# DerrickWang005/CRIS.pytorch

Hardware: AMD Instinct MI355X
Metric: train-step samples/sec, CRIS-R50 416x416 bs=64; loss parity vs ref (higher is better)
Workload: dtype bf16; 1 GPU; CRIS-R50 bf16 training step (fwd+BCE+bwd+Adam), 416x416, per-GPU bs=8, 17-token text, synthetic RefCOCO-shape batch resident in HBM (BASELINE.json configs[1]); global_batch=8, parallelism=dp1, launch=graph, graph_captured=True, syncbn_exchange=none, grad_exchange=none

## Files before the change

### cris/pytorch_amd/csrc/api.hip

```cpp
#include "common.h"
#include "../../../include/cris_hip.h"
#include <stdarg.h>
#include <string.h>

static thread_local char g_err[512] = {0};

void cris_set_error(const char* fmt, ...) {
    va_list ap;
    va_start(ap, fmt);
    vsnprintf(g_err, sizeof(g_err), fmt, ap);
    va_end(ap);
}

extern "C" const char* cris_last_error(void) { return g_err; }
extern "C" int cris_abi_version(void) { return CRIS_ABI_VERSION; }

extern "C" int cris_sizeof(const char* name) {
#define S(n) if (!strcmp(name, #n)) return (int)sizeof(n)
    S(cris_conv_gemm_params);
    S(cris_wgrad_params);
    S(cris_conv_gemm_group);
    S(cris_wgrad_group);
    S(cris_pack_desc);
    S(cris_conv_gemm_fp8_params);
    S(cris_pack_fp8_desc);
    S(cris_bn_apply_params);
    S(cris_bn_bwd_params);
    S(cris_ln_fwd_params);
    S(cris_ln_bwd_params);
    S(cris_sum_entry);
    S(cris_sum_group);
    S(cris_attn_params);
    S(cris_adam_desc);
    S(cris_ema_desc);
    S(cris_p2p_params);
    S(cris_p2p_link);
    S(cris_p2p_arena_params);
    S(cris_zero_ranges);
    S(cris_sample_desc);
    S(cris_eval_desc);
    S(cris_jpeg_info);
    S(cris_jpeg_image);
#undef S
    return -1;
// ... 51 lines not shown
```

### cris/pytorch_amd/csrc/norm.hip

```cpp
#include "common.h"
#include "../../../include/cris_hip.h"
#include "p2p_ll.h"
#include <string.h>

#define BN_WIDE_MIN 128
#define BN_MERGE_MIN 512
#define BN_MERGE_SLICES 64

template <int PL>
__device__ __forceinline__ float bn_lane_sum(float (*sh)[17], float v, int pl, int cl) {
    __syncthreads();
    sh[pl][cl] = v;
    __syncthreads();
    if (PL == 64) {
        float g = 0.f;
        if (pl < 8) {
#pragma unroll
            for (int j = 0; j < 8; ++j) g += sh[pl * 8 + j][cl];
        }
        __syncthreads();
        if (pl < 8) sh[pl][cl] = g;
        __syncthreads();
    }
    float t = sh[0][cl];
// ... 1000 lines not shown
                if (in_relu && !(v[i][j] > 0.f)) m = 0.f;
                if (in_thresh) m = cris_keep(in_key, row * (uint32_t)C + (uint32_t)(c0 + j), in_thresh) ? m * in_scale : 0.f;
                v[i][j] *= m;
                if (WANT_MASK) mask_out[i][j] = m;
            }
        } else {
#pragma unroll
            for (int j = 0; j < 8; ++j) {
                v[i][j] = 0.f;
                if (WANT_MASK) mask_out[i][j] = 0.f;
            }
        }
    }
}

__global__ __launch_bounds__(256) void ln_fwd_kernel(const cris_ln_fwd_params p) {
    const int lane = threadIdx.x & 63;
    const int wave_g = blockIdx.x * 4 + (threadIdx.x >> 6);
    const int nwaves = gridDim.x * 4;
    const uint32_t sdev = p.seed_dev ? p.seed_dev[0] : 0u;
    const uint32_t in_key = cris_drop_key(p.in_seed + sdev, p.in_stream);
    const uint32_t out_key = cris_drop_key(p.out_seed + sdev, p.out_stream);
    const float in_scale = p.in_thresh ? 1.f / (1.f - p.in_drop_p) : 1.f;
    const float out_scale = p.out_thresh ? 1.f / (1.f - p.out_drop_p) : 1.f;
    const float invC = 1.f / (float)p.C;
    for (int row = wave_g; row < p.rows; row += nwaves) {
        float v[LN_MAXV][8];
        ln_load_row<false>(p.x, p.x_f32, (size_t)row * p.ldx, p.C, lane, p.in_relu, p.in_thresh, in_scale, in_key, (uint32_t)row,
                           v, v);
        float s = 0.f;
#pragma unroll
        for (int i = 0; i < LN_MAXV; ++i)
#pragma unroll
            for (int j = 0; j < 8; ++j) s += v[i][j];
        const float mean = wave_sum(s) * invC;
        float q = 0.f;
#pragma unroll
        for (int i = 0; i < LN_MAXV; ++i) {
            const int c0 = (lane + 64 * i) * 8;
            if (c0 < p.C) {
#pragma unroll
                for (int j = 0; j < 8; ++j) {
                    const float d = v[i][j] - mean;
                    q += d * d;
                }
            }
        }
        const float rstd = rsqrtf(wave_sum(q) * invC + p.eps);
        if (lane == 0) {
            p.mean[row] = mean;
            p.rstd[row] = rstd;
        }
#pragma unroll
        for (int i = 0; i < LN_MAXV; ++i) {
            const int c0 = (lane + 64 * i) * 8;
            if (c0 >= p.C) continue;
            float ga[8], be[8], o[8];
            load8f(p.gamma + c0, ga);
            load8f(p.beta + c0, be);
#pragma unroll
            for (int j = 0; j < 8; ++j) o[j] = (v[i][j] - mean) * rstd * ga[j] + be[j];
            const size_t oo = (size_t)row * p.C + c0;
            if (p.y) cris_st16(p.y + oo, pack8(o));
            if (p.ypos) {
                float pe[8], t[8];
                load8f(p.pos + (size_t)(row % p.pos_rows) * p.C + c0, pe);
#pragma unroll
                for (int j = 0; j < 8; ++j) t[j] = o[j] + pe[j];
                cris_st16(p.ypos + oo, pack8(t));
            }
            if (p.out_f32) {
                float r[8];
                if (p.resid) load8f(p.resid + oo, r);
                else {
#pragma unroll
                    for (int j = 0; j < 8; ++j) r[j] = 0.f;
                }
#pragma unroll
                for (int j = 0; j < 8; ++j) {
                    float t = o[j];
                    if (p.out_thresh) t = cris_keep(out_key, (uint32_t)row * (uint32_t)p.C + (uint32_t)(c0 + j), p.out_thresh) ? t * out_scale : 0.f;
                    r[j] += t;
                }
                *reinterpret_cast<float4*>(p.out_f32 + oo) = make_float4(r[0], r[1], r[2], r[3]);
                *reinterpret_cast<float4*>(p.out_f32 + oo + 4) = make_float4(r[4], r[5], r[6], r[7]);
            }
        }
    }
}

extern "C" int cris_ln_fwd(const cris_ln_fwd_params* pp, void* stream) {
    const cris_ln_fwd_params& p = *pp;
    CRIS_CHECK_ARG(p.x && p.gamma && p.beta && p.mean && p.rstd && p.rows > 0, "null operand");
    CRIS_CHECK_ARG((p.C & 7) == 0 && p.C <= 64 * 8 * LN_MAXV && (p.ldx & 7) == 0, "C must be a multiple of 8, <= 2048");
    CRIS_CHECK_ARG(!p.ypos || (p.pos && p.pos_rows > 0), "ypos needs pos");
    CRIS_CHECK_ARG((long)p.rows * p.C < (1L << 32), "dropout index overflow");
    const int grid = cris_grid_1d(p.rows, 4, 2048);
    hipLaunchKernelGGL(ln_fwd_kernel, dim3(grid), dim3(256), 0, (hipStream_t)stream, p);
    CRIS_LAUNCH_CHECK();
    return 0;
}

template <int V>
__global__ __launch_bounds__(256) void ln_bwd_kernel(const cris_ln_bwd_params p) {
    __shared__ float sg[2][64 * 8 * V];
    const int lane = threadIdx.x & 63;
    const int wave_g = blockIdx.x * 4 + (threadIdx.x >> 6);
    const int nwaves = gridDim.x * 4;
    for (int i = threadIdx.x; i < 2 * 64 * 8 * V; i += 256) (&sg[0][0])[i] = 0.f;
    __syncthreads();
    const uint32_t sdev = p.seed_dev ? p.seed_dev[0] : 0u;
    const uint32_t in_key = cris_drop_key(p.in_seed + sdev, p.in_stream);
    const uint32_t out_key = cris_drop_key(p.out_seed + sdev, p.out_stream);
    const float in_scale = p.in_thresh ? 1.f / (1.f - p.in_drop_p) : 1.f;
    const float out_scale = p.out_thresh ? 1.f / (1.f - p.out_drop_p) : 1.f;
// ... 27 lines not shown
                if (p.dypos) {
                    load8bf(p.dypos + oo, t);
#pragma unroll
                    for (int j = 0; j < 8; ++j) g[j] += t[j];
                }
                if (p.dout_f32) {
                    load8f(p.dout_f32 + oo, t);
#pragma unroll
                    for (int j = 0; j < 8; ++j) {
                        float d = t[j];
                        if (p.out_thresh) d = cris_keep(out_key, (uint32_t)row * (uint32_t)p.C + (uint32_t)(c0 + j), p.out_thresh) ? d * out_scale : 0.f;
                        g[j] += d;
                    }
                }
                load8f(p.gamma + c0, ga);
#pragma unroll
                for (int j = 0; j < 8; ++j) {
                    const float xh = (v[i][j] - mean) * rstd;
                    v[i][j] = xh;
                    dga[i][j] += g[j] * xh;
                    dbe[i][j] += g[j];
                    a[i][j] = g[j] * ga[j];
                    s1 += a[i][j];
                    s2 += a[i][j] * xh;
                }
            } else {
#pragma unroll
                for (int j = 0; j < 8; ++j) a[i][j] = 0.f;
            }
        }
        const float m1 = wave_sum(s1) * invC, m2 = wave_sum(s2) * invC;
#pragma unroll
        for (int i = 0; i < V; ++i) {
            const int c0 = (lane + 64 * i) * 8;
            if (c0 >= p.C) continue;
            float o[8];
#pragma unroll
            for (int j = 0; j < 8; ++j) o[j] = rstd * (a[i][j] - m1 - v[i][j] * m2) * msk[i][j];
            const size_t xo = (size_t)row * p.ldx + c0;
            if (p.dx_f32) {
                float* d = reinterpret_cast<float*>(p.dx) + xo;
                if (p.dx_accum) {
                    float old[8];
                    load8f(d, old);
#pragma unroll
                    for (int j = 0; j < 8; ++j) o[j] += old[j];
                }
                *reinterpret_cast<float4*>(d) = make_float4(o[0], o[1], o[2], o[3]);
                *reinterpret_cast<float4*>(d + 4) = make_float4(o[4], o[5], o[6], o[7]);
            } else {
                cris_st16(reinterpret_cast<bf16_t*>(p.dx) + xo, pack8(o));
            }
        }
    }
    for (int w = 0; w < 4; ++w) {
        if ((int)(threadIdx.x >> 6) == w) {
#pragma unroll
            for (int i = 0; i < V; ++i) {
                const int c0 = (lane + 64 * i) * 8;
                if (c0 < p.C) {
#pragma unroll
                    for (int j = 0; j < 8; ++j) {
                        sg[0][c0 + j] += dga[i][j];
                        sg[1][c0 + j] += dbe[i][j];
                    }
                }
            }
        }
        __syncthreads();
    }
    float* part = p.part + (size_t)blockIdx.x * 2 * p.C;
    for (int c = threadIdx.x; c < p.C; c += 256) {
        part[c] = sg[0][c];
        part[p.C + c] = sg[1][c];
    }
}

constexpr int LN_BWD_BLOCKS = 512;
static int ln_bwd_grid(int rows) { return cris_grid_1d(rows, 4, LN_BWD_BLOCKS); }
extern "C" int cris_ln_bwd_parts(int rows) { return ln_bwd_grid(rows); }

extern "C" int cris_ln_bwd(const cris_ln_bwd_params* pp, void* stream) {
    const cris_ln_bwd_params& p = *pp;
    CRIS_CHECK_ARG(p.x && p.gamma && p.mean && p.rstd && p.dx && p.part && p.rows > 0, "null operand");
    CRIS_CHECK_ARG(p.dy || p.dypos || p.dout_f32, "no incoming gradient");
    CRIS_CHECK_ARG((p.C & 7) == 0 && p.C <= 64 * 8 * LN_MAXV && (p.ldx & 7) == 0, "C must be a multiple of 8, <= 2048");
    CRIS_CHECK_ARG(!p.dx_accum || p.dx_f32, "accumulate only into fp32");
    static const int narrow = cris_env_int("CRIS_LN_BWD_V", 1);
    const dim3 grid(ln_bwd_grid(p.rows));
    if (narrow && p.C <= 512) hipLaunchKernelGGL(ln_bwd_kernel<1>, grid, dim3(256), 0, (hipStream_t)stream, p);
    else if (narrow && p.C <= 1024) hipLaunchKernelGGL(ln_bwd_kernel<2>, grid, dim3(256), 0, (hipStream_t)stream, p);
    else hipLaunchKernelGGL(ln_bwd_kernel<LN_MAXV>, grid, dim3(256), 0, (hipStream_t)stream, p);
    CRIS_LAUNCH_CHECK();
    return 0;
}

__global__ __launch_bounds__(256) void sum_group_kernel(const cris_sum_group g) {
    __shared__ float sh[4][64];
    int ei = 0;
#pragma unroll
    for (int i = 1; i < CRIS_SUM_GROUP_MAX; ++i) ei += g.block_start[i] <= (int)blockIdx.x ? 1 : 0;
    const cris_sum_entry e = g.e[ei];
    const int cl = threadIdx.x & 63, pl = threadIdx.x >> 6;
    const int c = (blockIdx.x - g.block_start[ei]) * 64 + cl;
    float a = 0.f;
    if (c < e.ncol)
        for (int i = pl; i < e.nparts; i += 4) a += e.part[(size_t)i * e.ld + c];
    sh[pl][cl] = a;
    __syncthreads();
    if (pl == 0 && c < e.ncol) e.out[c] = (sh[0][cl] + sh[1][cl]) + (sh[2][cl] + sh[3][cl]);
}
// ... 16 lines not shown
```

### cris/pytorch_amd/engine.py

```python
from __future__ import annotations

from typing import Callable, Dict, List, Optional

import torch
from torch import nn

from . import debug, ops, tables
from .arch import ClipSpec, HeadSpec, build_param_tree
from .ops import BF16, Drop, Geom, NO_DROP, pad8, pad32

F32 = torch.float32
BN_EPS, BN_MOM, LN_EPS = 1e-5, 0.1, 1e-5


class Act:
    __slots__ = ("t", "Bn", "H", "W", "C", "ld", "coff", "root", "_g", "aux")
    _engine = None

    def __init__(self, t, Bn, H, W, C, ld=None, coff=0, root=None):
        self.t, self.Bn, self.H, self.W, self.C = t, Bn, H, W, C
        self.ld = ld if ld is not None else C
        self.coff = coff
        self.root = root if root is not None else self
        self._g = None
# ... 443 lines not shown
                        ops.axpy_f32(resid.root._g, outs.g, 1.0)
                if dx_stream is not None:
                    dx, accum = dx_stream.grad_target()
                else:
                    dx, acc = x.grad_target()
                    accum = False
                    assert not acc, "bf16 LN input gradient cannot be accumulated"
                ops.ln_bwd(x.t, gamma, mean, rstd, rows, C, dx, ldx=x.ld, dy=None if (y is None or y.g is None) else y.g,
                           dypos=None if (ypos is None or ypos.g is None) else ypos.g,
                           dout_f32=None if outs is None else outs.g, dgamma=self.G[pfx + ".weight"], dbeta=self.G[pfx + ".bias"],
                           dx_accum=accum, in_relu=in_relu, in_drop=in_drop, out_drop=out_drop, queue=self._sq)

            self.tape.append(bwd)
        return y, ypos, outs

    def new_T(self, B, Hn, L, secs=1):
        Lpad = pad32(L)
        buf = self.zeros(secs, B * Hn * 64, Lpad, dtype=BF16)
        return dict(buf=buf, L=L, Lpad=Lpad, E=Hn * 64, sec_stride=B * Hn * 64 * Lpad)

    def attention(self, q: Act, k: Act, v: Act, Qt, Kt, Vt, B, Hn, Lq, Lk, *, causal=False, key_tokens=None, drop: Drop = NO_DROP):
        E = Hn * 64
        o = self.new_act(B, Lq, 1, E)
        lse = self.empty(B * Hn, Lq, dtype=F32)
        Lkp, Lqp = pad32(Lk), pad32(Lq)
        qv, kv, vv = q.t[:, q.coff:], k.t[:, k.coff:], v.t[:, v.coff:]
        prm = ops.attn_params(qv, kv, vv, Vt, B, Hn, Lq, Lk, Lkp, 64 ** -0.5, ldq=q.ld, ldk=k.ld, ldv=v.ld, Kt=Kt, Qt=Qt,
                              Lq_pad=Lqp, key_tokens=key_tokens, causal=causal, drop=drop)
        ops.attn_fwd(prm, o.t, lse, ldo=o.ld)
        if self.training:
# ... 329 lines not shown
                gx, acc = txt.grad_target()
                ops.add_bf16(txtpos.g, gx, txt.M, txt.C, b=gx if acc else None)
            self.tape.append(bwd_txtpos)
        for i in range(hd.num_layers):
            p = "decoder.layers.%d" % i
            v2, qk, _ = self.ln(vis, p + ".norm1", pos=vpos, pos_rows=HW, dx_stream=vis)
            T2, Tv = self.new_T(B, Hn, HW, secs=2), self.new_T(B, Hn, HW)
            G = self.group_begin()
            qkp = self.gemm(qk, p + ".self_attn.in_proj_weight", 2 * C, rows=(0, 2 * C), bias=p + ".self_attn.in_proj_bias", outT=T2, group=G)
            vp = self.gemm(v2, p + ".self_attn.in_proj_weight", C, rows=(2 * C, 3 * C), bias=p + ".self_attn.in_proj_bias", outT=Tv, group=G)
            self.group_end(G)
            o, dOt = self.attention(qkp.slice(0, C), qkp.slice(C, C), vp, T2["buf"][0], T2["buf"][1], Tv["buf"][0], B, Hn, HW, HW,
                                    drop=self.drop(i, 0))
            a = self.gemm(o, p + ".self_attn.out_proj.weight", C, bias=p + ".self_attn.out_proj.bias")
            self._patch_outT_on_dgrad(dOt)
            _, _, vis1 = self.ln(a, p + ".self_attn_norm", want_y=False, resid=vis, out_drop=self.drop(i, 1))
            _, qc, _ = self.ln(vis1, p + ".norm2", want_y=False, pos=vpos, pos_rows=HW, dx_stream=vis1)
            Tq, Tk, Tvv = self.new_T(B, Hn, HW), self.new_T(B, Hn, L), self.new_T(B, Hn, L)
            m = p + ".multihead_attn"
            G = self.group_begin()
            qx = self.gemm(qc, m + ".in_proj_weight", C, rows=(0, C), bias=m + ".in_proj_bias", outT=Tq, group=G)
            kx = self.gemm(txtpos, m + ".in_proj_weight", C, rows=(C, 2 * C), bias=m + ".in_proj_bias", outT=Tk, group=G)
            vx = self.gemm(txt, m + ".in_proj_weight", C, rows=(2 * C, 3 * C), bias=m + ".in_proj_bias", outT=Tvv, group=G)
            self.group_end(G)
            o2, dOt2 = self.attention(qx, kx, vx, Tq["buf"][0], Tk["buf"][0], Tvv["buf"][0], B, Hn, HW, L, key_tokens=word,
                                      drop=self.drop(i, 2))
            a2 = self.gemm(o2, m + ".out_proj.weight", C, bias=m + ".out_proj.bias")
            self._patch_outT_on_dgrad(dOt2)
            _, _, vis2 = self.ln(a2, p + ".cross_attn_norm", want_y=False, resid=vis1, out_drop=self.drop(i, 3))
            h3, _, _ = self.ln(vis2, p + ".norm3", dx_stream=vis2)
            u = self.gemm(h3, p + ".ffn.0.weight", hd.dim_ffn, bias=p + ".ffn.0.bias")
            hn, _, _ = self.ln(u, p + ".ffn.3", in_relu=True, in_drop=self.drop(i, 4))
            vis3 = self.new_act(B, H, W, C, dtype=F32)
            self.gemm(hn, p + ".ffn.4.weight", C, bias=p + ".ffn.4.bias", out=vis3, resid=vis2, drop=self.drop(i, 5), stream_grad=vis3)
            self._link_stream(vis3, vis2)
            vis = vis3
        out, _, _ = self.ln(vis, "decoder.norm", dx_stream=vis)
        if self.training:
            def bwd_in():
                gx, acc = fq.grad_target()
                assert not acc
                ops.cast_f32_bf16(vis0.g, gx)
            self.tape.insert(self._dec_tape_start, bwd_in)
        return out

# ... 187 lines not shown
```

### cris/pytorch_amd/hip.py

```python
import contextlib
import ctypes as C
import os

import torch

_HERE = os.path.dirname(os.path.abspath(__file__))
LIB_PATH = os.path.join(_HERE, "csrc", "libcris_hip.so")
if os.environ.get("CRIS_LIB_VARIANT"):
    LIB_PATH = os.path.join(_HERE, "csrc", "variants", "libcris_hip_%s.so" % os.environ["CRIS_LIB_VARIANT"])

P, I, L, F, U = C.c_void_p, C.c_int, C.c_long, C.c_float, C.c_uint32


class ConvGemmParams(C.Structure):
    _fields_ = [("A", P), ("Wt", P), ("bias", P), ("resid", P), ("out", P), ("outT", P), ("colsum", P), ("colsq", P),
                ("T_sec_stride", L),
                ("lda", I), ("a_coff", I),
                ("Bn", I), ("H", I), ("W", I), ("C", I),
                ("OH", I), ("OW", I), ("KH", I), ("KW", I), ("stride", I), ("pad", I),
                ("ldb", I),
                ("M", I), ("N", I), ("K", I),
                ("act", I),
                ("ldr", I), ("r_coff", I), ("resid_f32", I),
                ("ldc", I), ("c_coff", I), ("out_f32", I),
# ... 99 lines not shown
                ("out_drop_p", F), ("out_thresh", U), ("out_seed", U), ("out_stream", U),
                ("eps", F),
                ("seed_dev", P)]


class LnBwdParams(C.Structure):
    _fields_ = [("x", P), ("x_f32", I), ("ldx", I),
                ("gamma", P),
                ("mean", P), ("rstd", P),
                ("dy", P), ("dypos", P), ("dout_f32", P),
                ("part", P),
                ("dx", P), ("dx_f32", I), ("dx_accum", I),
                ("rows", I), ("C", I),
                ("in_relu", I),
                ("in_drop_p", F), ("in_thresh", U), ("in_seed", U), ("in_stream", U),
                ("out_drop_p", F), ("out_thresh", U), ("out_seed", U), ("out_stream", U),
                ("seed_dev", P)]


class AttnParams(C.Structure):
    _fields_ = [("Q", P), ("ldq", I),
                ("K", P), ("ldk", I),
                ("V", P), ("ldv", I),
                ("Vt", P), ("Kt", P), ("Qt", P), ("Lk_pad", I), ("Lq_pad", I),
                ("key_tokens", P),
                ("O", P), ("ldo", I),
                ("lse", P),
                ("dO", P), ("lddo", I), ("dOt", P),
                ("delta", P),
                ("dQ", P), ("lddq", I),
# ... 77 lines not shown

class P2PLink(C.Structure):
    _fields_ = [("boxes", P), ("err", P), ("gen_dev", P),
                ("gen_host", I), ("rank", I), ("world", I),
                ("slot", I), ("slots", I), ("max_floats", I), ("spin_limit", I)]


class P2PArenaParams(C.Structure):
    _fields_ = [("arenas", P), ("lo", C.c_long), ("n", C.c_long), ("link", P2PLink), ("blocks", I)]


STRUCTS = {
    "cris_conv_gemm_params": ConvGemmParams, "cris_conv_gemm_group": ConvGemmGroup, "cris_wgrad_params": WgradParams, "cris_wgrad_group": WgradGroup, "cris_pack_desc": PackDesc,
    "cris_conv_gemm_fp8_params": ConvGemmFp8Params, "cris_pack_fp8_desc": PackFp8Desc,
    "cris_bn_apply_params": BnApplyParams, "cris_bn_bwd_params": BnBwdParams, "cris_ln_fwd_params": LnFwdParams,
    "cris_ln_bwd_params": LnBwdParams, "cris_sum_entry": SumEntry, "cris_sum_group": SumGroup, "cris_attn_params": AttnParams, "cris_adam_desc": AdamDesc, "cris_ema_desc": EmaDesc, "cris_p2p_params": P2PParams, "cris_p2p_link": P2PLink, "cris_p2p_arena_params": P2PArenaParams, "cris_zero_ranges": ZeroRanges,
    "cris_sample_desc": SampleDesc, "cris_eval_desc": EvalDesc, "cris_jpeg_info": JpegInfo, "cris_jpeg_image": JpegImage,
}

_SIGS = {
    "cris_last_error": (C.c_char_p, []),
    "cris_abi_version": (I, []),
    "cris_sizeof": (I, [C.c_char_p]),
    "cris_echo_conv_gemm": (L, [P]),
    "cris_conv_gemm": (I, [P, P]),
    "cris_conv_wgrad": (I, [P, P]),
    "cris_conv_wgrad_group": (I, [P, P]),
    "cris_conv_wgrad_tile": (I, [P]),
    "cris_wgrad_reduce": (I, [P, P]),
    "cris_wgrad_reduce_group": (I, [P, P]),
    "cris_wgrad_ws_floats": (L, [I, I, I, I]),
# ... 18 lines not shown
    "cris_absmax_ws_floats": (I, []),
    "cris_bn_partials_rows": (I, [I]),
    "cris_bn_finalize": (I, [P, P, I, I, F, F, P, P, P, P, F, F, I, P, P, P, P, P, P, P]),
    "cris_bn_sync_pack": (I, [P, P, P, F, I, P]),
    "cris_bn_sync_unpack": (I, [P, P, F, I, P]),
    "cris_colstats_bf16": (I, [P, I, I, I, I, I, P, P, P]),
    "cris_bn_eval_coeffs": (I, [P, P, P, P, F, I, P, P, P]),
    "cris_bn_apply": (I, [P, P]),
    "cris_bn_bwd_reduce": (I, [P, P]),
    "cris_bn_bwd_apply": (I, [P, P]),
    "cris_bn_bwd_ws_floats": (L, [P]),
    "cris_ln_bwd_parts": (I, [I]),
    "cris_sum_tables": (I, [P, P]),
    "cris_ln_fwd": (I, [P, P]),
    "cris_ln_bwd": (I, [P, P]),
    "cris_attn_fwd": (I, [P, P]),
    "cris_attn_bwd_dq": (I, [P, P]),
    "cris_attn_bwd_dkv": (I, [P, P]),
    "cris_attn_plan": (I, [P, I]),
    "cris_stem_im2col": (I, [P, I, I, I, P, P]),
    "cris_avgpool2_fwd": (I, [P, I, I, I, I, I, I, P, I, I, P]),
    "cris_avgpool2_bwd": (I, [P, I, I, I, I, I, I, P, I, I, I, P]),
    "cris_upsample2_fwd": (I, [P, I, I, I, I, I, I, P, I, I, P]),
    "cris_upsample2_bwd": (I, [P, I, I, I, I, I, I, P, I, I, I, P]),
    "cris_fill_coords": (I, [P, I, I, I, I, I, I, P]),
    "cris_gather_samples_bf16": (I, [P, I, I, P, I, I, I, P, I, I, P]),
    "cris_add_bf16": (I, [P, I, I, P, I, I, P, I, I, I, I, P]),
    "cris_add_rowtable": (I, [P, I, P, I, P, I, I, I, P]),
    "cris_cast_f32_bf16": (I, [P, P, L, P]),
    "cris_cast_bf16_f32": (I, [P, P, L, I, P]),
# ... 181 lines not shown
```

### cris/pytorch_amd/ops.py

```python
from __future__ import annotations

import ctypes as C
import math
import os
from dataclasses import dataclass
from typing import Optional

import torch

from . import hip
from .hip import ptr

BF16 = torch.bfloat16


def _stream():
    return torch.cuda.current_stream().cuda_stream


def pad8(n: int) -> int:
    return (n + 7) // 8 * 8


def pad32(n: int) -> int:
# ... 568 lines not shown
    p.dx, p.dx_f32, p.dx_accum = ptr(dx), int(dx.dtype == torch.float32), int(dx_accum)
    p.rows, p.C, p.in_relu = rows, C_, int(in_relu)
    p.in_drop_p, p.in_thresh, p.in_seed, p.in_stream = in_drop.p, in_drop.thresh, in_drop.seed & 0xFFFFFFFF, in_drop.stream
    p.out_drop_p, p.out_thresh, p.out_seed, p.out_stream = out_drop.p, out_drop.thresh, out_drop.seed & 0xFFFFFFFF, out_drop.stream
    p.seed_dev = ptr(in_drop.dev if in_drop.dev is not None else out_drop.dev)
    hip.call("cris_ln_bwd", C.byref(p), _stream())
    q = queue if queue is not None else SumQueue()
    if dgamma is not None:
        q.add(part, dgamma, nparts, C_, 2 * C_, 0)
    if dbeta is not None:
        q.add(part, dbeta, nparts, C_, 2 * C_, C_)
    if queue is None:
        q.flush()


def attn_params(Q, K, V, Vt, B, Hn, Lq, Lk, Lk_pad, scale, *, ldq=None, ldk=None, ldv=None, Kt=None, Qt=None, Lq_pad=0,
                key_tokens=None, causal=False, drop: Drop = NO_DROP):
    p = hip.AttnParams()
    p.Q, p.ldq = ptr(Q), ldq if ldq is not None else Q.shape[-1]
    p.K, p.ldk = ptr(K), ldk if ldk is not None else K.shape[-1]
    p.V, p.ldv = ptr(V), ldv if ldv is not None else V.shape[-1]
    p.Vt, p.Kt, p.Qt, p.Lk_pad, p.Lq_pad = ptr(Vt), ptr(Kt), ptr(Qt), Lk_pad, Lq_pad
    p.key_tokens = ptr(key_tokens)
    p.B, p.Hn, p.Lq, p.Lk, p.causal, p.scale = B, Hn, Lq, Lk, int(causal), float(scale)
    p.drop_p, p.drop_thresh, p.drop_seed, p.drop_stream = drop.p, drop.thresh, drop.seed & 0xFFFFFFFF, drop.stream
    p.drop_seed_dev = ptr(drop.dev)
    return p


def attn_fwd(p, O, lse, ldo=None):
# ... 666 lines not shown
```

### include/cris_hip.h

```cpp
#ifndef CRIS_HIP_H
#define CRIS_HIP_H
#include <stddef.h>
#include <stdint.h>
#ifdef __cplusplus
extern "C" {
#endif

typedef uint16_t cris_bf16;

const char* cris_last_error(void);
#define CRIS_ABI_VERSION 8
int cris_abi_version(void);
int cris_sizeof(const char* struct_name);
long cris_echo_conv_gemm(const void* conv_gemm_params);

typedef struct {
    const cris_bf16* A;
    const cris_bf16* Wt;
    const float* bias;
    const void* resid;
    void* out;
    cris_bf16* outT;
    float* colsum;
    float* colsq;
// ... 191 lines not shown
    const float* gamma;
    const float* mean; const float* rstd;
    const cris_bf16* dy;
    const cris_bf16* dypos;
    const float* dout_f32;
    float* part;
    void* dx; int dx_f32; int dx_accum;
    int rows, C;
    int in_relu;
    float in_drop_p; uint32_t in_thresh, in_seed, in_stream;
    float out_drop_p; uint32_t out_thresh, out_seed, out_stream;
    const uint32_t* seed_dev;
} cris_ln_bwd_params;
int cris_ln_bwd(const cris_ln_bwd_params* p, void* stream);
int cris_ln_bwd_parts(int rows);

#define CRIS_SUM_GROUP_MAX 64
typedef struct { const float* part; float* out; int nparts, ncol, ld, pad_; } cris_sum_entry;
typedef struct {
    int n;
    int block_start[CRIS_SUM_GROUP_MAX + 1];
    cris_sum_entry e[CRIS_SUM_GROUP_MAX];
} cris_sum_group;
int cris_sum_tables(const cris_sum_group* g, void* stream);

typedef struct {
    const cris_bf16* Q;  int ldq;
    const cris_bf16* K;  int ldk;
    const cris_bf16* V;  int ldv;
    const cris_bf16* Vt; const cris_bf16* Kt; const cris_bf16* Qt; int Lk_pad, Lq_pad;
// ... 271 lines not shown
```

Measured before the change: 670.3 samples/s.

## Fuse residual LayerNorm pair into one kernel and specialize LN forward by width

Adds fused forward and backward kernels that run a residual-add LayerNorm followed directly by the next LayerNorm in one pass. The residual stream stays in registers between the two norms, which saves a launch and a round trip of the fp32 stream through HBM. The decoder layer now uses this fused pair for cross_attn_norm plus norm3. LN forward is also templated on the vector count per lane, with occupancy hints and gamma/beta/resid loaded early for narrow C. This adds register pressure and a second set of partial dgamma/dbeta buffers in backward.

```diff
diff --git a/cris/pytorch_amd/csrc/api.hip b/cris/pytorch_amd/csrc/api.hip
--- a/cris/pytorch_amd/csrc/api.hip
+++ b/cris/pytorch_amd/csrc/api.hip
@@ -28,6 +28,8 @@
     S(cris_bn_bwd_params);
     S(cris_ln_fwd_params);
     S(cris_ln_bwd_params);
+    S(cris_ln_pair_fwd_params);
+    S(cris_ln_pair_bwd_params);
     S(cris_sum_entry);
     S(cris_sum_group);
     S(cris_attn_params);
diff --git a/cris/pytorch_amd/csrc/norm.hip b/cris/pytorch_amd/csrc/norm.hip
--- a/cris/pytorch_amd/csrc/norm.hip
+++ b/cris/pytorch_amd/csrc/norm.hip
@@ -1038,7 +1038,65 @@
     }
 }
 
-__global__ __launch_bounds__(256) void ln_fwd_kernel(const cris_ln_fwd_params p) {
+template <int V>
+__device__ __forceinline__ void ln_row_stats(const float (&v)[V][8], int C, int lane, float invC, float eps, float& mean, float& rstd) {
+    float s = 0.f;
+#pragma unroll
+    for (int i = 0; i < V; ++i)
+#pragma unroll
+        for (int j = 0; j < 8; ++j) s += v[i][j];
+    mean = wave_sum(s) * invC;
+    float q = 0.f;
+#pragma unroll
+    for (int i = 0; i < V; ++i) {
+        const int c0 = (lane + 64 * i) * 8;
+        if (c0 < C) {
+#pragma unroll
+            for (int j = 0; j < 8; ++j) {
+                const float d = v[i][j] - mean;
+                q += d * d;
+            }
+        }
+    }
+    rstd = rsqrtf(wave_sum(q) * invC + eps);
+}
+
+__device__ __forceinline__ void ln_affine(const float (&v)[8], float mean, float rstd, const float (&ga)[8], const float (&be)[8], float (&o)[8]) {
+#pragma unroll
+    for (int j = 0; j < 8; ++j) o[j] = (v[j] - mean) * rstd * ga[j] + be[j];
+}
+
+__device__ __forceinline__ void ln_resid_add(const float (&o)[8], float (&r)[8], uint32_t out_key, uint32_t idx0, uint32_t out_thresh, float out_scale) {
+#pragma unroll
+    for (int j = 0; j < 8; ++j) {
+        float t = o[j];
+        if (out_thresh) t = cris_keep(out_key, idx0 + (uint32_t)j, out_thresh) ? t * out_scale : 0.f;
+        r[j] += t;
+    }
+}
+
+__device__ __forceinline__ void ln_store8f(float* d, const float (&r)[8]) {
+    *reinterpret_cast<float4*>(d) = make_float4(r[0], r[1], r[2], r[3]);
+    *reinterpret_cast<float4*>(d + 4) = make_float4(r[4], r[5], r[6], r[7]);
+}
+
+__device__ __forceinline__ void ln_fwd_operands(const cris_ln_fwd_params& p, int row, int lane, int i, float (&ga)[8], float (&be)[8],
+                                                float (&r)[8]) {
+    const int c0 = (lane + 64 * i) * 8;
+    const int cc = c0 < p.C ? c0 : 0;
+    load8f(p.gamma + cc, ga);
+    load8f(p.beta + cc, be);
+    if (p.out_f32 && p.resid) load8f(p.resid + (size_t)row * p.C + cc, r);
+    else {
+#pragma unroll
+        for (int j = 0; j < 8; ++j) r[j] = 0.f;
+    }
+}
+
+#define LN_FWD_EARLY(V) ((V) <= 2)
+#define LN_FWD_WAVES(V) ((V) == 1 ? 6 : (V) == 2 ? 4 : 5)
+template <int V>
+__global__ __launch_bounds__(256, LN_FWD_WAVES(V)) void ln_fwd_kernel(const cris_ln_fwd_params p) {
     const int lane = threadIdx.x & 63;
     const int wave_g = blockIdx.x * 4 + (threadIdx.x >> 6);
     const int nwaves = gridDim.x * 4;
@@ -1049,41 +1107,30 @@
     const float out_scale = p.out_thresh ? 1.f / (1.f - p.out_drop_p) : 1.f;
     const float invC = 1.f / (float)p.C;
     for (int row = wave_g; row < p.rows; row += nwaves) {
-        float v[LN_MAXV][8];
-        ln_load_row<false>(p.x, p.x_f32, (size_t)row * p.ldx, p.C, lane, p.in_relu, p.in_thresh, in_scale, in_key, (uint32_t)row,
-                           v, v);
-        float s = 0.f;
-#pragma unroll
-        for (int i = 0; i < LN_MAXV; ++i)
-#pragma unroll
-            for (int j = 0; j < 8; ++j) s += v[i][j];
-        const float mean = wave_sum(s) * invC;
-        float q = 0.f;
-#pragma unroll
-        for (int i = 0; i < LN_MAXV; ++i) {
-            const int c0 = (lane + 64 * i) * 8;
-            if (c0 < p.C) {
-#pragma unroll
-                for (int j = 0; j < 8; ++j) {
-                    const float d = v[i][j] - mean;
-                    q += d * d;
-                }
-            }
-        }
-        const float rstd = rsqrtf(wave_sum(q) * invC + p.eps);
+        float v[V][8];
+        ln_load_row<false, V>(p.x, p.x_f32, (size_t)row * p.ldx, p.C, lane, p.in_relu, p.in_thresh, in_scale, in_key, (uint32_t)row,
+                              v, v);
+        float ga[V][8], be[V][8], r[V][8];
+        if (LN_FWD_EARLY(V)) {
+#pragma unroll
+            for (int i = 0; i < V; ++i) ln_fwd_operands(p, row, lane, i, ga[i], be[i], r[i]);
+        }
+        float mean, rstd;
+        ln_row_stats<V>(v, p.C, lane, invC, p.eps, mean, rstd);
         if (lane == 0) {
             p.mean[row] = mean;
             p.rstd[row] = rstd;
         }
 #pragma unroll
-        for (int i = 0; i < LN_MAXV; ++i) {
+        for (int i = 0; i < V; ++i) {
             const int c0 = (lane + 64 * i) * 8;
             if (c0 >= p.C) continue;
-            float ga[8], be[8], o[8];
-            load8f(p.gamma + c0, ga);
-            load8f(p.beta + c0, be);
-#pragma unroll
-            for (int j = 0; j < 8; ++j) o[j] = (v[i][j] - mean) * rstd * ga[j] + be[j];
+            if (!LN_FWD_EARLY(V)) {
+                load8f(p.gamma + c0, ga[i]);
+                load8f(p.beta + c0, be[i]);
+            }
+            float o[8];
+            ln_affine(v[i], mean, rstd, ga[i], be[i], o);
             const size_t oo = (size_t)row * p.C + c0;
             if (p.y) cris_st16(p.y + oo, pack8(o));
             if (p.ypos) {
@@ -1094,35 +1141,177 @@
                 cris_st16(p.ypos + oo, pack8(t));
             }
             if (p.out_f32) {
-                float r[8];
-                if (p.resid) load8f(p.resid + oo, r);
-                else {
-#pragma unroll
-                    for (int j = 0; j < 8; ++j) r[j] = 0.f;
+                if (!LN_FWD_EARLY(V)) {
+                    if (p.resid) load8f(p.resid + oo, r[i]);
+                    else {
+#pragma unroll
+                        for (int j = 0; j < 8; ++j) r[i][j] = 0.f;
+                    }
                 }
-#pragma unroll
-                for (int j = 0; j < 8; ++j) {
-                    float t = o[j];
-                    if (p.out_thresh) t = cris_keep(out_key, (uint32_t)row * (uint32_t)p.C + (uint32_t)(c0 + j), p.out_thresh) ? t * out_scale : 0.f;
-                    r[j] += t;
-                }
-                *reinterpret_cast<float4*>(p.out_f32 + oo) = make_float4(r[0], r[1], r[2], r[3]);
-                *reinterpret_cast<float4*>(p.out_f32 + oo + 4) = make_float4(r[4], r[5], r[6], r[7]);
-            }
-        }
-    }
-}
+                ln_resid_add(o, r[i], out_key, (uint32_t)row * (uint32_t)p.C + (uint32_t)c0, p.out_thresh, out_scale);
+                ln_store8f(p.out_f32 + oo, r[i]);
+            }
+        }
+    }
+}
+
+static int ln_vecs(int C, int narrow) { return !narrow ? LN_MAXV : C <= 512 ? 1 : C <= 1024 ? 2 : LN_MAXV; }
 
 extern "C" int cris_ln_fwd(const cris_ln_fwd_params* pp, void* stream) {
     const cris_ln_fwd_params& p = *pp;
     CRIS_CHECK_ARG(p.x && p.gamma && p.beta && p.mean && p.rstd && p.rows > 0, "null operand");
-    CRIS_CHECK_ARG((p.C & 7) == 0 && p.C <= 64 * 8 * LN_MAXV && (p.ldx & 7) == 0, "C must be a multiple of 8, <= 2048");
+    CRIS_CHECK_ARG((p.C & 7) == 0 && p.C > 0 && p.C <= 64 * 8 * LN_MAXV && (p.ldx & 7) == 0, "C must be a multiple of 8, <= 2048");
     CRIS_CHECK_ARG(!p.ypos || (p.pos && p.pos_rows > 0), "ypos needs pos");
     CRIS_CHECK_ARG((long)p.rows * p.C < (1L << 32), "dropout index overflow");
-    const int grid = cris_grid_1d(p.rows, 4, 2048);
-    hipLaunchKernelGGL(ln_fwd_kernel, dim3(grid), dim3(256), 0, (hipStream_t)stream, p);
+    static const int narrow = cris_env_int("CRIS_LN_FWD_V", 1);
+    const dim3 grid(cris_grid_1d(p.rows, 4, 2048));
+    switch (ln_vecs(p.C, narrow)) {
+    case 1: hipLaunchKernelGGL(ln_fwd_kernel<1>, grid, dim3(256), 0, (hipStream_t)stream, p); break;
+    case 2: hipLaunchKernelGGL(ln_fwd_kernel<2>, grid, dim3(256), 0, (hipStream_t)stream, p); break;
+    default: hipLaunchKernelGGL(ln_fwd_kernel<LN_MAXV>, grid, dim3(256), 0, (hipStream_t)stream, p);
+    }
     CRIS_LAUNCH_CHECK();
     return 0;
+}
+
+__device__ __forceinline__ void ln_pair_operands(const cris_ln_pair_fwd_params& p, int row, int lane, int i, float (&ga)[8], float (&be)[8],
+                                                 float (&r)[8]) {
+    const int c0 = (lane + 64 * i) * 8;
+    const int cc = c0 < p.C ? c0 : 0;
+    load8f(p.gamma1 + cc, ga);
+    load8f(p.beta1 + cc, be);
+    load8f(p.resid + (size_t)row * p.C + cc, r);
+}
+
+#define LN_PAIR_FWD_WAVES(V) ((V) == 1 ? 5 : (V) == 2 ? 4 : 2)
+template <int V>
+__global__ __launch_bounds__(256, LN_PAIR_FWD_WAVES(V)) void ln_pair_fwd_kernel(const cris_ln_pair_fwd_params p) {
+    const int lane = threadIdx.x & 63;
+    const int wave_g = blockIdx.x * 4 + (threadIdx.x >> 6);
+    const int nwaves = gridDim.x * 4;
+    const uint32_t sdev = p.seed_dev ? p.seed_dev[0] : 0u;
+    const uint32_t out_key = cris_drop_key(p.out_seed + sdev, p.out_stream);
+    const float out_scale = p.out_thresh ? 1.f / (1.f - p.out_drop_p) : 1.f;
+    const float invC = 1.f / (float)p.C;
+    for (int row = wave_g; row < p.rows; row += nwaves) {
+        float v[V][8];
+        ln_load_row<false, V>(p.x, 0, (size_t)row * p.ldx, p.C, lane, 0, 0u, 1.f, 0u, (uint32_t)row, v, v);
+        float ga[V][8], be[V][8], r[V][8];
+        if (LN_FWD_EARLY(V)) {
+#pragma unroll
+            for (int i = 0; i < V; ++i) ln_pair_operands(p, row, lane, i, ga[i], be[i], r[i]);
+        }
+        float mean, rstd;
+        ln_row_stats<V>(v, p.C, lane, invC, p.eps, mean, rstd);
+        if (lane == 0) {
+            p.mean1[row] = mean;
+            p.rstd1[row] = rstd;
+        }
+#pragma unroll
+        for (int i = 0; i < V; ++i) {
+            const int c0 = (lane + 64 * i) * 8;
+            if (c0 < p.C) {
+                if (!LN_FWD_EARLY(V)) ln_pair_operands(p, row, lane, i, ga[i], be[i], r[i]);
+                float o[8];
+                ln_affine(v[i], mean, rstd, ga[i], be[i], o);
+                ln_resid_add(o, r[i], out_key, (uint32_t)row * (uint32_t)p.C + (uint32_t)c0, p.out_thresh, out_scale);
+                ln_store8f(p.stream + (size_t)row * p.C + c0, r[i]);
+            } else {
+#pragma unroll
+                for (int j = 0; j < 8; ++j) r[i][j] = 0.f;
+            }
+        }
+#pragma unroll
+        for (int i = 0; i < V; ++i) {
+            const int c0 = (lane + 64 * i) * 8;
+            const int cc = c0 < p.C ? c0 : 0;
+            load8f(p.gamma2 + cc, ga[i]);
+            load8f(p.beta2 + cc, be[i]);
+        }
+        ln_row_stats<V>(r, p.C, lane, invC, p.eps, mean, rstd);
+        if (lane == 0) {
+            p.mean2[row] = mean;
+            p.rstd2[row] = rstd;
+        }
+#pragma unroll
+        for (int i = 0; i < V; ++i) {
+            const int c0 = (lane + 64 * i) * 8;
+            if (c0 >= p.C) continue;
+            float o[8];
+            ln_affine(r[i], mean, rstd, ga[i], be[i], o);
+            const size_t oo = (size_t)row * p.C + c0;
+            if (p.y) cris_st16(p.y + oo, pack8(o));
+            if (p.ypos) {
+                float pe[8], t[8];
+                load8f(p.pos + (size_t)(row % p.pos_rows) * p.C + c0, pe);
+#pragma unroll
+                for (int j = 0; j < 8; ++j) t[j] = o[j] + pe[j];
+                cris_st16(p.ypos + oo, pack8(t));
+            }
+        }
+    }
+}
+
+extern "C" int cris_ln_pair_fwd(const cris_ln_pair_fwd_params* pp, void* stream) {
+    const cris_ln_pair_fwd_params& p = *pp;
+    CRIS_CHECK_ARG(p.x && p.gamma1 && p.beta1 && p.resid && p.stream && p.mean1 && p.rstd1 && p.rows > 0, "null operand");
+    CRIS_CHECK_ARG(p.gamma2 && p.beta2 && p.mean2 && p.rstd2 && (p.y || p.ypos), "null operand of the second norm");
+    CRIS_CHECK_ARG((p.C & 7) == 0 && p.C > 0 && p.C <= 64 * 8 * LN_MAXV && (p.ldx & 7) == 0 && p.ldx >= p.C, "C must be a multiple of 8, <= 2048");
+    CRIS_CHECK_ARG(!p.ypos || (p.pos && p.pos_rows > 0), "ypos needs pos");
+    CRIS_CHECK_ARG((long)p.rows * p.C < (1L << 32), "dropout index overflow");
+    const dim3 grid(cris_grid_1d(p.rows, 4, 2048));
+    switch (ln_vecs(p.C, 1)) {
+    case 1: hipLaunchKernelGGL(ln_pair_fwd_kernel<1>, grid, dim3(256), 0, (hipStream_t)stream, p); break;
+    case 2: hipLaunchKernelGGL(ln_pair_fwd_kernel<2>, grid, dim3(256), 0, (hipStream_t)stream, p); break;
+    default: hipLaunchKernelGGL(ln_pair_fwd_kernel<LN_MAXV>, grid, dim3(256), 0, (hipStream_t)stream, p);
+    }
+    CRIS_LAUNCH_CHECK();
+    return 0;
+}
+
+__device__ __forceinline__ void ln_bwd_vec(float (&v)[8], const float (&g)[8], const float (&ga)[8], float mean, float rstd,
+                                           float (&dga)[8], float (&dbe)[8], float (&a)[8], float& s1, float& s2) {
+#pragma unroll
+    for (int j = 0; j < 8; ++j) {
+        const float xh = (v[j] - mean) * rstd;
+        v[j] = xh;
+        dga[j] += g[j] * xh;
+        dbe[j] += g[j];
+        a[j] = g[j] * ga[j];
+        s1 += a[j];
+        s2 += a[j] * xh;
+    }
+}
+
+__device__ __forceinline__ void ln_bwd_dx(const float (&a)[8], const float (&xh)[8], const float (&msk)[8], float rstd, float m1, float m2,
+                                          float (&o)[8]) {
+#pragma unroll
+    for (int j = 0; j < 8; ++j) o[j] = rstd * (a[j] - m1 - xh[j] * m2) * msk[j];
+}
+
+template <int V>
+__device__ __forceinline__ void ln_bwd_flush(float* sga, float* sbe, const float (&dga)[V][8], const float (&dbe)[V][8], int C, int lane,
+                                             float* part) {
+    for (int w = 0; w < 4; ++w) {
+        if ((int)(threadIdx.x >> 6) == w) {
+#pragma unroll
+            for (int i = 0; i < V; ++i) {
+                const int c0 = (lane + 64 * i) * 8;
+                if (c0 < C) {
+#pragma unroll
+                    for (int j = 0; j < 8; ++j) {
+                        sga[c0 + j] += dga[i][j];
+                        sbe[c0 + j] += dbe[i][j];
+                    }
+                }
+            }
+        }
+        __syncthreads();
+    }
+    for (int c = threadIdx.x; c < C; c += 256) {
+        part[c] = sga[c];
+        part[C + c] = sbe[c];
+    }
 }
 
 template <int V>
@@ -1180,16 +1369,7 @@
                     }
                 }
                 load8f(p.gamma + c0, ga);
-#pragma unroll
-                for (int j = 0; j < 8; ++j) {
-                    const float xh = (v[i][j] - mean) * rstd;
-                    v[i][j] = xh;
-                    dga[i][j] += g[j] * xh;
-                    dbe[i][j] += g[j];
-                    a[i][j] = g[j] * ga[j];
-                    s1 += a[i][j];
-                    s2 += a[i][j] * xh;
-                }
+                ln_bwd_vec(v[i], g, ga, mean, rstd, dga[i], dbe[i], a[i], s1, s2);
             } else {
 #pragma unroll
                 for (int j = 0; j < 8; ++j) a[i][j] = 0.f;
@@ -1201,8 +1381,7 @@
             const int c0 = (lane + 64 * i) * 8;
             if (c0 >= p.C) continue;
             float o[8];
-#pragma unroll
-            for (int j = 0; j < 8; ++j) o[j] = rstd * (a[i][j] - m1 - v[i][j] * m2) * msk[i][j];
+            ln_bwd_dx(a[i], v[i], msk[i], rstd, m1, m2, o);
             const size_t xo = (size_t)row * p.ldx + c0;
             if (p.dx_f32) {
                 float* d = reinterpret_cast<float*>(p.dx) + xo;
@@ -1212,34 +1391,127 @@
 #pragma unroll
                     for (int j = 0; j < 8; ++j) o[j] += old[j];
                 }
-                *reinterpret_cast<float4*>(d) = make_float4(o[0], o[1], o[2], o[3]);
-                *reinterpret_cast<float4*>(d + 4) = make_float4(o[4], o[5], o[6], o[7]);
+                ln_store8f(d, o);
             } else {
                 cris_st16(reinterpret_cast<bf16_t*>(p.dx) + xo, pack8(o));
             }
         }
     }
-    for (int w = 0; w < 4; ++w) {
-        if ((int)(threadIdx.x >> 6) == w) {
+    ln_bwd_flush<V>(sg[0], sg[1], dga, dbe, p.C, lane, p.part + (size_t)blockIdx.x * 2 * p.C);
+}
+
+template <int V>
+__global__ __launch_bounds__(256, V == 1 ? 4 : 1) void ln_pair_bwd_kernel(const cris_ln_pair_bwd_params p) {
+    __shared__ float sg[4][64 * 8 * V];
+    const int lane = threadIdx.x & 63;
+    const int wave_g = blockIdx.x * 4 + (threadIdx.x >> 6);
+    const int nwaves = gridDim.x * 4;
+    for (int i = threadIdx.x; i < 4 * 64 * 8 * V; i += 256) (&sg[0][0])[i] = 0.f;
+    __syncthreads();
+    const uint32_t sdev = p.seed_dev ? p.seed_dev[0] : 0u;
+    const uint32_t out_key = cris_drop_key(p.out_seed + sdev, p.out_stream);
+    const float out_scale = p.out_thresh ? 1.f / (1.f - p.out_drop_p) : 1.f;
+    const float invC = 1.f / (float)p.C;
+    float dga1[V][8], dbe1[V][8], dga2[V][8], dbe2[V][8];
+#pragma unroll
+    for (int i = 0; i < V; ++i)
+#pragma unroll
+        for (int j = 0; j < 8; ++j) dga1[i][j] = dbe1[i][j] = dga2[i][j] = dbe2[i][j] = 0.f;
+
+    for (int row = wave_g; row < p.rows; row += nwaves) {
+        float ds[V][8];
+        float v1[V][8], msk1[V][8], old[V][8];
+        ln_load_row<true, V>(p.x, 0, (size_t)row * p.ldx, p.C, lane, 0, 0u, 1.f, 0u, (uint32_t)row, v1, msk1);
+        const float mean1 = p.mean1[row], rstd1 = p.rstd1[row];
+        if (p.dstream_accum) {
+#pragma unroll
+            for (int i = 0; i < V; ++i) {
+                const int c0 = (lane + 64 * i) * 8;
+                load8f(p.dstream + (size_t)row * p.C + (c0 < p.C ? c0 : 0), old[i]);
+            }
+        }
+        {
+            float v[V][8], msk[V][8], a[V][8];
+            ln_load_row<true, V>(p.stream, 1, (size_t)row * p.C, p.C, lane, 0, 0u, 1.f, 0u, (uint32_t)row, v, msk);
+            const float mean = p.mean2[row], rstd = p.rstd2[row];
+            float s1 = 0.f, s2 = 0.f;
 #pragma unroll
             for (int i = 0; i < V; ++i) {
                 const int c0 = (lane + 64 * i) * 8;
                 if (c0 < p.C) {
+                    const size_t oo = (size_t)row * p.C + c0;
+                    float g[8], t[8], ga[8];
+#pragma unroll
+                    for (int j = 0; j < 8; ++j) g[j] = 0.f;
+                    if (p.dy) {
+                        load8bf(p.dy + oo, t);
+#pragma unroll
+                        for (int j = 0; j < 8; ++j) g[j] += t[j];
+                    }
+                    if (p.dypos) {
+                        load8bf(p.dypos + oo, t);
+#pragma unroll
+                        for (int j = 0; j < 8; ++j) g[j] += t[j];
+                    }
+                    load8f(p.gamma2 + c0, ga);
+                    ln_bwd_vec(v[i], g, ga, mean, rstd, dga2[i], dbe2[i], a[i], s1, s2);
+                } else {
+#pragma unroll
+                    for (int j = 0; j < 8; ++j) a[i][j] = 0.f;
+                }
+            }
+            const float m1 = wave_sum(s1) * invC, m2 = wave_sum(s2) * invC;
+#pragma unroll
+            for (int i = 0; i < V; ++i) {
+                const int c0 = (lane + 64 * i) * 8;
+                if (c0 >= p.C) continue;
+                ln_bwd_dx(a[i], v[i], msk[i], rstd, m1, m2, ds[i]);
+                float* d = p.dstream + (size_t)row * p.C + c0;
+                if (p.dstream_accum) {
+#pragma unroll
+                    for (int j = 0; j < 8; ++j) ds[i][j] += old[i][j];
+                }
+                ln_store8f(d, ds[i]);
+            }
+        }
+        {
+            float (&v)[V][8] = v1, (&msk)[V][8] = msk1;
+            float a[V][8];
+            const float mean = mean1, rstd = rstd1;
+            float s1 = 0.f, s2 = 0.f;
+#pragma unroll
+            for (int i = 0; i < V; ++i) {
+                const int c0 = (lane + 64 * i) * 8;
+                if (c0 < p.C) {
+                    float g[8], ga[8];
+#pragma unroll
+                    for (int j = 0; j < 8; ++j) g[j] = 0.f;
 #pragma unroll
                     for (int j = 0; j < 8; ++j) {
-                        sg[0][c0 + j] += dga[i][j];
-                        sg[1][c0 + j] += dbe[i][j];
+                        float d = ds[i][j];
+                        if (p.out_thresh) d = cris_keep(out_key, (uint32_t)row * (uint32_t)p.C + (uint32_t)(c0 + j), p.out_thresh) ? d * out_scale : 0.f;
+                        g[j] += d;
                     }
+                    load8f(p.gamma1 + c0, ga);
+                    ln_bwd_vec(v[i], g, ga, mean, rstd, dga1[i], dbe1[i], a[i], s1, s2);
+                } else {
+#pragma unroll
+                    for (int j = 0; j < 8; ++j) a[i][j] = 0.f;
                 }
             }
-        }
-        __syncthreads();
-    }
-    float* part = p.part + (size_t)blockIdx.x * 2 * p.C;
-    for (int c = threadIdx.x; c < p.C; c += 256) {
-        part[c] = sg[0][c];
-        part[p.C + c] = sg[1][c];
-    }
+            const float m1 = wave_sum(s1) * invC, m2 = wave_sum(s2) * invC;
+#pragma unroll
+            for (int i = 0; i < V; ++i) {
+                const int c0 = (lane + 64 * i) * 8;
+                if (c0 >= p.C) continue;
+                float o[8];
+                ln_bwd_dx(a[i], v[i], msk[i], rstd, m1, m2, o);
+                cris_st16(p.dx + (size_t)row * p.ldx + c0, pack8(o));
+            }
+        }
+    }
+    ln_bwd_flush<V>(sg[0], sg[1], dga1, dbe1, p.C, lane, p.part1 + (size_t)blockIdx.x * 2 * p.C);
+    ln_bwd_flush<V>(sg[2], sg[3], dga2, dbe2, p.C, lane, p.part2 + (size_t)blockIdx.x * 2 * p.C);
 }
 
 constexpr int LN_BWD_BLOCKS = 512;
@@ -1261,6 +1533,24 @@
     return 0;
 }
 
+extern "C" int cris_ln_pair_bwd(const cris_ln_pair_bwd_params* pp, void* stream) {
+    const cris_ln_pair_bwd_params& p = *pp;
+    CRIS_CHECK_ARG(p.x && p.gamma1 && p.mean1 && p.rstd1 && p.dx && p.part1 && p.rows > 0, "null operand");
+    CRIS_CHECK_ARG(p.stream && p.gamma2 && p.mean2 && p.rstd2 && p.dstream && p.part2, "null operand of the second norm");
+    CRIS_CHECK_ARG(p.dy || p.dypos, "no incoming gradient");
+    CRIS_CHECK_ARG((p.C & 7) == 0 && p.C > 0 && p.C <= 64 * 8 * LN_MAXV && (p.ldx & 7) == 0 && p.ldx >= p.C, "C must be a multiple of 8, <= 2048");
+    CRIS_CHECK_ARG((long)p.rows * p.C < (1L << 32), "dropout index overflow");
+    static const int narrow = cris_env_int("CRIS_LN_BWD_V", 1);
+    const dim3 grid(ln_bwd_grid(p.rows));
+    switch (ln_vecs(p.C, narrow)) {
+    case 1: hipLaunchKernelGGL(ln_pair_bwd_kernel<1>, grid, dim3(256), 0, (hipStream_t)stream, p); break;
+    case 2: hipLaunchKernelGGL(ln_pair_bwd_kernel<2>, grid, dim3(256), 0, (hipStream_t)stream, p); break;
+    default: hipLaunchKernelGGL(ln_pair_bwd_kernel<LN_MAXV>, grid, dim3(256), 0, (hipStream_t)stream, p);
+    }
+    CRIS_LAUNCH_CHECK();
+    return 0;
+}
+
 __global__ __launch_bounds__(256) void sum_group_kernel(const cris_sum_group g) {
     __shared__ float sh[4][64];
     int ei = 0;
diff --git a/cris/pytorch_amd/engine.py b/cris/pytorch_amd/engine.py
--- a/cris/pytorch_amd/engine.py
+++ b/cris/pytorch_amd/engine.py
@@ -481,6 +481,36 @@
             self.tape.append(bwd)
         return y, ypos, outs
 
+    def ln_pair(self, x: Act, pfx1: str, resid: Act, out_drop: Drop, pfx2: str, *, want_y=True, pos=None, pos_rows=0):
+        rows, C = x.M, x.C
+        g1, b1, g2, b2 = (self.P[k] for k in (pfx1 + ".weight", pfx1 + ".bias", pfx2 + ".weight", pfx2 + ".bias"))
+        mean1, rstd1 = self.empty(rows, dtype=F32), self.empty(rows, dtype=F32)
+        outs = self.new_act(x.Bn, x.H, x.W, C, dtype=F32)
+        mean2, rstd2 = self.empty(rows, dtype=F32), self.empty(rows, dtype=F32)
+        y = self.new_act(x.Bn, x.H, x.W, C) if want_y else None
+        ypos = self.new_act(x.Bn, x.H, x.W, C) if pos is not None else None
+        ops.ln_pair_fwd(x.t, g1, b1, resid.t, outs.t, mean1, rstd1, g2, b2, mean2, rstd2, rows, C, ldx=x.ld,
+                        y=None if y is None else y.t, ypos=None if ypos is None else ypos.t, pos=pos, pos_rows=pos_rows,
+                        out_drop=out_drop, eps=LN_EPS)
+        if y is not None:
+            y.aux["ln_stats"] = (mean2, rstd2)
+        if self.training:
+            def bwd():
+                ds, accum = outs.grad_target()
+                dx, acc = x.grad_target()
+                assert not acc, "bf16 LN input gradient cannot be accumulated"
+                ops.ln_pair_bwd(x.t, g1, mean1, rstd1, outs.t, g2, mean2, rstd2, rows, C, dx, ds, ldx=x.ld,
+                                dy=None if (y is None or y.g is None) else y.g, dypos=None if (ypos is None or ypos.g is None) else ypos.g,
+                                dstream_accum=accum, dgamma1=self.G[pfx1 + ".weight"], dbeta1=self.G[pfx1 + ".bias"],
+                                dgamma2=self.G[pfx2 + ".weight"], dbeta2=self.G[pfx2 + ".bias"], out_drop=out_drop, queue=self._sq)
+                if resid.root._g is None:
+                    resid.root._g = outs.g
+                elif resid.root._g is not outs.g:
+                    ops.axpy_f32(resid.root._g, outs.g, 1.0)
+
+            self.tape.append(bwd)
+        return y, ypos, outs
+
     def new_T(self, B, Hn, L, secs=1):
         Lpad = pad32(L)
         buf = self.zeros(secs, B * Hn * 64, Lpad, dtype=BF16)
@@ -840,8 +870,7 @@
                                     drop=self.drop(i, 0))
             a = self.gemm(o, p + ".self_attn.out_proj.weight", C, bias=p + ".self_attn.out_proj.bias")
             self._patch_outT_on_dgrad(dOt)
-            _, _, vis1 = self.ln(a, p + ".self_attn_norm", want_y=False, resid=vis, out_drop=self.drop(i, 1))
-            _, qc, _ = self.ln(vis1, p + ".norm2", want_y=False, pos=vpos, pos_rows=HW, dx_stream=vis1)
+            _, qc, vis1 = self.ln_pair(a, p + ".self_attn_norm", vis, self.drop(i, 1), p + ".norm2", want_y=False, pos=vpos, pos_rows=HW)
             Tq, Tk, Tvv = self.new_T(B, Hn, HW), self.new_T(B, Hn, L), self.new_T(B, Hn, L)
             m = p + ".multihead_attn"
             G = self.group_begin()
@@ -853,8 +882,7 @@
                                       drop=self.drop(i, 2))
             a2 = self.gemm(o2, m + ".out_proj.weight", C, bias=m + ".out_proj.bias")
             self._patch_outT_on_dgrad(dOt2)
-            _, _, vis2 = self.ln(a2, p + ".cross_attn_norm", want_y=False, resid=vis1, out_drop=self.drop(i, 3))
-            h3, _, _ = self.ln(vis2, p + ".norm3", dx_stream=vis2)
+            h3, _, vis2 = self.ln_pair(a2, p + ".cross_attn_norm", vis1, self.drop(i, 3), p + ".norm3")
             u = self.gemm(h3, p + ".ffn.0.weight", hd.dim_ffn, bias=p + ".ffn.0.bias")
             hn, _, _ = self.ln(u, p + ".ffn.3", in_relu=True, in_drop=self.drop(i, 4))
             vis3 = self.new_act(B, H, W, C, dtype=F32)
diff --git a/cris/pytorch_amd/hip.py b/cris/pytorch_amd/hip.py
--- a/cris/pytorch_amd/hip.py
+++ b/cris/pytorch_amd/hip.py
@@ -137,6 +137,36 @@
                 ("rows", I), ("C", I),
                 ("in_relu", I),
                 ("in_drop_p", F), ("in_thresh", U), ("in_seed", U), ("in_stream", U),
+                ("out_drop_p", F), ("out_thresh", U), ("out_seed", U), ("out_stream", U),
+                ("seed_dev", P)]
+
+
+class LnPairFwdParams(C.Structure):
+    _fields_ = [("x", P), ("ldx", I),
+                ("gamma1", P), ("beta1", P),
+                ("resid", P),
+                ("stream", P),
+                ("mean1", P), ("rstd1", P),
+                ("gamma2", P), ("beta2", P),
+                ("pos", P), ("pos_rows", I),
+                ("y", P), ("ypos", P),
+                ("mean2", P), ("rstd2", P),
+                ("rows", I), ("C", I),
+                ("out_drop_p", F), ("out_thresh", U), ("out_seed", U), ("out_stream", U),
+                ("eps", F),
+                ("seed_dev", P)]
+
+
+class LnPairBwdParams(C.Structure):
+    _fields_ = [("x", P), ("ldx", I),
+                ("gamma1", P), ("mean1", P), ("rstd1", P),
+                ("stream", P),
+                ("gamma2", P), ("mean2", P), ("rstd2", P),
+                ("dy", P), ("dypos", P),
+                ("dstream", P), ("dstream_accum", I),
+                ("dx", P),
+                ("part1", P), ("part2", P),
+                ("rows", I), ("C", I),
                 ("out_drop_p", F), ("out_thresh", U), ("out_seed", U), ("out_stream", U),
                 ("seed_dev", P)]
 
@@ -244,7 +274,7 @@
     "cris_conv_gemm_params": ConvGemmParams, "cris_conv_gemm_group": ConvGemmGroup, "cris_wgrad_params": WgradParams, "cris_wgrad_group": WgradGroup, "cris_pack_desc": PackDesc,
     "cris_conv_gemm_fp8_params": ConvGemmFp8Params, "cris_pack_fp8_desc": PackFp8Desc,
     "cris_bn_apply_params": BnApplyParams, "cris_bn_bwd_params": BnBwdParams, "cris_ln_fwd_params": LnFwdParams,
-    "cris_ln_bwd_params": LnBwdParams, "cris_sum_entry": SumEntry, "cris_sum_group": SumGroup, "cris_attn_params": AttnParams, "cris_adam_desc": AdamDesc, "cris_ema_desc": EmaDesc, "cris_p2p_params": P2PParams, "cris_p2p_link": P2PLink, "cris_p2p_arena_params": P2PArenaParams, "cris_zero_ranges": ZeroRanges,
+    "cris_ln_bwd_params": LnBwdParams, "cris_ln_pair_fwd_params": LnPairFwdParams, "cris_ln_pair_bwd_params": LnPairBwdParams, "cris_sum_entry": SumEntry, "cris_sum_group": SumGroup, "cris_attn_params": AttnParams, "cris_adam_desc": AdamDesc, "cris_ema_desc": EmaDesc, "cris_p2p_params": P2PParams, "cris_p2p_link": P2PLink, "cris_p2p_arena_params": P2PArenaParams, "cris_zero_ranges": ZeroRanges,
     "cris_sample_desc": SampleDesc, "cris_eval_desc": EvalDesc, "cris_jpeg_info": JpegInfo, "cris_jpeg_image": JpegImage,
 }
 
@@ -293,6 +323,8 @@
     "cris_sum_tables": (I, [P, P]),
     "cris_ln_fwd": (I, [P, P]),
     "cris_ln_bwd": (I, [P, P]),
+    "cris_ln_pair_fwd": (I, [P, P]),
+    "cris_ln_pair_bwd": (I, [P, P]),
     "cris_attn_fwd": (I, [P, P]),
     "cris_attn_bwd_dq": (I, [P, P]),
     "cris_attn_bwd_dkv": (I, [P, P]),
diff --git a/cris/pytorch_amd/ops.py b/cris/pytorch_amd/ops.py
--- a/cris/pytorch_amd/ops.py
+++ b/cris/pytorch_amd/ops.py
@@ -606,6 +606,51 @@
         q.flush()
 
 
+def ln_pair_fwd(x, gamma1, beta1, resid, stream, mean1, rstd1, gamma2, beta2, mean2, rstd2, rows, C_, *, ldx=None, y=None, ypos=None,
+                pos=None, pos_rows=0, out_drop: Drop = NO_DROP, eps=1e-5):
+    p = hip.LnPairFwdParams()
+    p.x, p.ldx = ptr(x), ldx if ldx is not None else C_
+    p.gamma1, p.beta1, p.resid, p.stream, p.mean1, p.rstd1 = ptr(gamma1), ptr(beta1), ptr(resid), ptr(stream), ptr(mean1), ptr(rstd1)
+    p.gamma2, p.beta2, p.mean2, p.rstd2 = ptr(gamma2), ptr(beta2), ptr(mean2), ptr(rstd2)
+    p.pos, p.pos_rows, p.y, p.ypos = ptr(pos), pos_rows, ptr(y), ptr(ypos)
+    p.rows, p.C = rows, C_
+    p.out_drop_p, p.out_thresh, p.out_seed, p.out_stream = out_drop.p, out_drop.thresh, out_drop.seed & 0xFFFFFFFF, out_drop.stream
+    p.seed_dev = ptr(out_drop.dev)
+    p.eps = eps
+    if x.dtype != torch.bfloat16:
+        raise ValueError("ln_pair_fwd: the first norm's input is bf16")
+    hip.call("cris_ln_pair_fwd", C.byref(p), _stream())
+
+
+def ln_pair_bwd(x, gamma1, mean1, rstd1, stream, gamma2, mean2, rstd2, rows, C_, dx, dstream, *, ldx=None, dy=None, dypos=None,
+                dstream_accum=False, dgamma1=None, dbeta1=None, dgamma2=None, dbeta2=None, out_drop: Drop = NO_DROP,
+                queue: Optional[SumQueue] = None):
+    p = hip.LnPairBwdParams()
+    p.x, p.ldx = ptr(x), ldx if ldx is not None else C_
+    p.gamma1, p.mean1, p.rstd1 = ptr(gamma1), ptr(mean1), ptr(rstd1)
+    p.stream, p.gamma2, p.mean2, p.rstd2 = ptr(stream), ptr(gamma2), ptr(mean2), ptr(rstd2)
+    p.dy, p.dypos = ptr(dy), ptr(dypos)
+    p.dstream, p.dstream_accum, p.dx = ptr(dstream), int(dstream_accum), ptr(dx)
+    nparts = hip.load().cris_ln_bwd_parts(rows)
+    part2 = torch.empty(nparts, 2 * C_, dtype=torch.float32, device=x.device)
+    part1 = torch.empty(nparts, 2 * C_, dtype=torch.float32, device=x.device)
+    p.part1, p.part2 = ptr(part1), ptr(part2)
+    p.rows, p.C = rows, C_
+    p.out_drop_p, p.out_thresh, p.out_seed, p.out_stream = out_drop.p, out_drop.thresh, out_drop.seed & 0xFFFFFFFF, out_drop.stream
+    p.seed_dev = ptr(out_drop.dev)
+    if x.dtype != torch.bfloat16 or dx.dtype != torch.bfloat16 or dstream.dtype != torch.float32:
+        raise ValueError("ln_pair_bwd: x and dx are bf16, dstream fp32")
+    hip.call("cris_ln_pair_bwd", C.byref(p), _stream())
+    q = queue if queue is not None else SumQueue()
+    for part, dg, db in ((part2, dgamma2, dbeta2), (part1, dgamma1, dbeta1)):
+        if dg is not None:
+            q.add(part, dg, nparts, C_, 2 * C_, 0)
+        if db is not None:
+            q.add(part, db, nparts, C_, 2 * C_, C_)
+    if queue is None:
+        q.flush()
+
+
 def attn_params(Q, K, V, Vt, B, Hn, Lq, Lk, Lk_pad, scale, *, ldq=None, ldk=None, ldv=None, Kt=None, Qt=None, Lq_pad=0,
                 key_tokens=None, causal=False, drop: Drop = NO_DROP):
     p = hip.AttnParams()
diff --git a/include/cris_hip.h b/include/cris_hip.h
--- a/include/cris_hip.h
+++ b/include/cris_hip.h
@@ -229,6 +229,40 @@
 } cris_ln_bwd_params;
 int cris_ln_bwd(const cris_ln_bwd_params* p, void* stream);
 int cris_ln_bwd_parts(int rows);
+
+typedef struct {
+    const cris_bf16* x; int ldx;
+    const float* gamma1; const float* beta1;
+    const float* resid;
+    float* stream;
+    float* mean1; float* rstd1;
+    const float* gamma2; const float* beta2;
+    const float* pos; int pos_rows;
+    cris_bf16* y;
+    cris_bf16* ypos;
+    float* mean2; float* rstd2;
+    int rows, C;
+    float out_drop_p; uint32_t out_thresh, out_seed, out_stream;
+    float eps;
+    const uint32_t* seed_dev;
+} cris_ln_pair_fwd_params;
+int cris_ln_pair_fwd(const cris_ln_pair_fwd_params* p, void* stream);
+
+typedef struct {
+    const cris_bf16* x; int ldx;
+    const float* gamma1; const float* mean1; const float* rstd1;
+    const float* stream;
+    const float* gamma2; const float* mean2; const float* rstd2;
+    const cris_bf16* dy;
+    const cris_bf16* dypos;
+    float* dstream; int dstream_accum;
+    cris_bf16* dx;
+    float* part1; float* part2;
+    int rows, C;
+    float out_drop_p; uint32_t out_thresh, out_seed, out_stream;
+    const uint32_t* seed_dev;
+} cris_ln_pair_bwd_params;
+int cris_ln_pair_bwd(const cris_ln_pair_bwd_params* p, void* stream);
 
 #define CRIS_SUM_GROUP_MAX 64
 typedef struct { const float* part; float* out; int nparts, ncol, ld, pad_; } cris_sum_entry;
```

Measured after the change: 675.5 samples/s (median of 6 runs). About the same (+0.8%).
